# maiziezhoulab/FocalSV

Measured on AMD Instinct MI355X. Metric: target regions/sec (50 kb, 30x HiFi), higher is better.
Workload: dtype u32; 1 GPU; 256 synthetic 50 kb regions per GPU, 30x HiFi-like reads U(10k,20k), 0.2% error, seed 1000+i (BASELINE.json configs[1]); regions_per_gpu=256

## Files before the change

focalsv_amd/csrc/asm.hip:

```cpp
#include "asm_kernels.h"
#include "k_kmer.h"
#include "layout.h"
#include <algorithm>
#include <chrono>
#include <cstdio>
#include <cstdlib>
#include <cstring>
#include <vector>
#include <thread>
#include <atomic>

namespace {

enum { KN_SKETCH, KN_UNIQ, KN_CHAIN, KN_BPM, KN_RESCUE, KN_PATH_FAST, KN_PATH_DP, KN_CONSENSUS, KN_REPACK, KN_EXACT, KN_STITCH, KN_PARTITION, KN_BND, KN_BND_CONS,
       KN_UNIQ_LONG, KN_CHAIN_SPILL,
       KN_CONS_DEEP, KN_BND_DEEP,
       KN_COUNT,
       ST_SKETCH = KN_COUNT, ST_CHAIN, ST_VERIFY, ST_PATH, ST_CONSENSUS, ST_FINAL };
const char *const kn_names[KN_COUNT] = {"k_sketch", "k_uniq", "k_chain", "k5_bpm", "k_rescue_accept", "k_path_fast", "k_path_dp", "k_consensus",
                                        "k_repack", "k_exact", "k_stitch", "k_partition", "k_bnd_tasks", "k_bnd_consensus", "k_uniq_long", "k_chain_spill",
                                        "k_consensus_deep", "k_bnd_consensus_deep"};
static_assert(KN_COUNT <= FSV_MAX_KERNEL_STATS, "fsv_asm_stats holds every kernel's row");
enum { PASS_NONE = -1, PASS_WINDOWS, PASS_JUNCTIONS, PASS_BCIG, PASS_COUNT };

// ... 910 lines not shown
    BcigArgs BA;
    BA.tasks = W.tasks.p; BA.paths = W.paths.p; BA.n_tasks = R.ct + CT_TASKS;
    BA.pair_read = W.pair_read.p; BA.read_dirty = W.read_dirty.p; BA.gwin_off = W.gwin_off.p;
    BA.thr_tab = W.thr_tab.p; BA.k_cap = P.k_cap;
    BA.tasks2 = W.tasks2.p; BA.bc_idx = W.bc_idx.p; BA.n_tasks2 = ct3 + CT_TASKS;
    BA.n_same = ct3 + CT_B_RETRY; BA.n_used = ct3 + CT_B_LIST;
    BA.res2 = W.res2.p; BA.paths2 = W.paths2.p; BA.bc_rec = W.bc_rec.p; BA.bc_win = W.bc_win.p;
    W.kt.begin(ctx, KN_PARTITION, 0);
    FSV_LAUNCH(ctx, ctx->stream, k_bcig_tasks, dim3((fsv_grid_for(task_cap, 256) + 7u) & ~7u), dim3(256), 0, BA);
    W.kt.end(ctx);
    W.kt.begin(ctx, PASS_BCIG, KN_BPM, 0);
    TRY(fsv_bpm_windows_dev_n(ctx, R.store, W.tasks2.p, task_cap, ct3 + CT_TASKS, W.res2.p, P.k_cap));
    W.kt.end(ctx);
    TRY(path_stage(ctx, W, PathJob{R.store, W.tasks2.p, W.res2.p, W.paths2.p, task_cap, ct3 + CT_TASKS, ct3, PASS_BCIG, R.round, R.wide_bands, P.k_cap, false}));
    W.kt.begin(ctx, KN_PARTITION, 0);
    FSV_LAUNCH(ctx, ctx->stream, k_bcig_accept, dim3(fsv_grid_for(task_cap, 256)), dim3(256), 0, BA);
    W.kt.end(ctx);
    SA.bc_idx = W.bc_idx.p; SA.bc_rec = W.bc_rec.p; SA.bc_paths = W.paths2.p;
    SL.bc_win = W.bc_win.p;
    return FSV_OK;
}

static int consensus_stage(fsv_ctx *ctx, AsmWs &W, Round &R)
{
    const fsv_asm_params &P = R.P; const Batch &B = R.B;
    const uint32_t n_gwin = R.n_gwin;
    TRY(consensus_setup(ctx, W, R));
    const ConsArgs &C = R.C;
    const bool partition = B.n_pairs && P.partition;
    SiteArgs SA{};
    SiteLists SL{};
    if (partition) TRY(partition_setup(ctx, W, R, SA, SL));
    if (partition && P.junction_cigars) TRY(junction_cigars(ctx, W, R, SA, SL));
    const dim3 grid_w((n_gwin + 7u) & ~7u);
    W.kt.begin(ctx, PASS_WINDOWS, KN_CONSENSUS, (uint64_t)n_gwin * (96 + 448));
    if (R.wide_bands) {
        if (partition) FSV_LAUNCH(ctx, ctx->stream, (k_consensus<FSV_EV_CAP_WIDE, 1>), grid_w, dim3(64), 0, C, n_gwin, SL);
        else FSV_LAUNCH(ctx, ctx->stream, (k_consensus<FSV_EV_CAP_WIDE, 0>), grid_w, dim3(64), 0, C, n_gwin, SL);
    } else {
        if (partition) FSV_LAUNCH(ctx, ctx->stream, (k_consensus<FSV_EV_CAP, 1>), grid_w, dim3(64), 0, C, n_gwin, SL);
        else FSV_LAUNCH(ctx, ctx->stream, (k_consensus<FSV_EV_CAP, 0>), grid_w, dim3(64), 0, C, n_gwin, SL);
    }
    W.kt.end(ctx);
    if (partition) {
        const uint32_t grid_l = std::min<uint32_t>(std::max(1u, n_gwin), (uint32_t)ctx->n_cu * 16);
        W.kt.begin(ctx, KN_PARTITION, (uint64_t)B.n_reads * 4);
        FSV_LAUNCH(ctx, ctx->stream, k_snp_sites, dim3(grid_l), dim3(64), 0, C, SA, SL);
        FSV_LAUNCH(ctx, ctx->stream, k_hap_partition, dim3(B.n_reads), dim3(64), 0, C, SA, W.ovl.p, W.ovl_c.p, SL);
        if (R.wide_bands) FSV_LAUNCH(ctx, ctx->stream, k_consensus_redo<FSV_EV_CAP_WIDE>, dim3(grid_l), dim3(64), 0, C, SL);
        else FSV_LAUNCH(ctx, ctx->stream, k_consensus_redo<FSV_EV_CAP>, dim3(grid_l), dim3(64), 0, C, SL);
        W.kt.end(ctx);
    }
    if (C.deep_list) {
        W.kt.begin(ctx, KN_CONS_DEEP, 0);
        FSV_LAUNCH(ctx, ctx->stream, k_consensus_deep, dim3(R.deep_grid), dim3(64), 0, C, SL, R.deep);
        W.kt.end(ctx);
    }
    return FSV_OK;
}

static int finish_round(fsv_ctx *ctx, AsmWs &W, Round &R)
{
    const fsv_asm_params &P = R.P; const Batch &B = R.B;
    const uint32_t n_gwin = R.n_gwin;
    TRY(ensure(ctx, W.lb, std::max(1u, n_gwin)));
    FSV_LAUNCH(ctx, ctx->stream, k_newlen, dim3(fsv_grid_for(B.n_reads, 256)), dim3(256), 0, W.gwin_off.p, W.cwin_len.p, B.n_reads, W.new_len.p, W.lb.p);
    std::vector<int32_t> nlen(B.n_reads);
    TRY(download(ctx, nlen.data(), W.new_len, B.n_reads));
    for (int pass = 0; pass < PASS_COUNT; pass++)
        FSV_HIP(ctx, hipMemcpyAsync(R.h_ct.data() + (size_t)R.row(pass) * CT_SLOT, W.ct_of(R.row(pass)), CT_SLOT * 4, hipMemcpyDeviceToHost, ctx->stream));
    FSV_HIP(ctx, hipStreamSynchronize(ctx->stream));
    if (R.h_ct[(size_t)R.round * CT_SLOT + CT_OVERFLOW]) return fsv_fail(ctx, FSV_ECAP, "internal window task buffer overflow");
    Geometry G2;
    TRY(make_geometry(ctx, B, nlen, G2, P.w, &R.mz_fixed));
    Dev<uint32_t> &dst = W.store[R.round & 1];
    const uint32_t total_words = G2.word_off[B.n_reads];
    TRY(ensure(ctx, dst, (size_t)total_words + 8));
    TRY(upload(ctx, W.unpack_off, G2.word_off));
    W.kt.begin(ctx, KN_REPACK, (uint64_t)n_gwin * 384 + (uint64_t)total_words * 4);
    FSV_LAUNCH(ctx, ctx->stream, k_repack, dim3(B.n_reads), dim3(256), 0, W.gwin_off.p, W.lb.p, W.cwin.p, W.unpack_off.p, W.new_len.p, B.n_reads,
               R.round + 1 < P.n_rounds ? 1 : 0, dst.p);
    W.kt.end(ctx);
    FSV_HIP(ctx, hipMemsetAsync(dst.p + total_words, 0, 32, ctx->stream));
    R.store = dst.p;
    R.len = nlen;
    for (int32_t l : R.len) if (l >= 65536) R.short_reads = false;
    R.G = G2;
    return FSV_OK;
}

struct SetLayout { std::vector<std::vector<Piece>> contigs; bool fallback = false; };
struct Final {
    std::vector<uint32_t> hit_first, hwarn, h_setcols;
    const fsv_hit *hraw = nullptr;
    bool any_inexact = false;
    std::vector<SetLayout> lay;
    uint64_t used = 0;
    Trace trace;
};

static int begin_final(fsv_ctx *ctx, AsmWs &W, Round &R)
{
    R.ct = W.ct_of(R.P.n_rounds); R.task_cap = 0;
    TRY(upload(ctx, W.word_off, R.G.word_off));
    TRY(upload(ctx, W.len, R.len));
    TRY(upload(ctx, W.mz_off, R.G.mz_off));
    TRY(ensure(ctx, W.tasks, 2));
    return FSV_OK;
}

static int rechain_listed(fsv_ctx *ctx, AsmWs &W, const Round &R, const uint32_t *n_list_dev)
{
    const fsv_asm_params &P = R.P; const Batch &B = R.B;
    ChainArgs A2 = W.last_chain;
// ... 1036 lines not shown
```

focalsv_amd/csrc/asm_kernels.h:

```cpp
#pragma once
#include "bpm_device.h"
#include "k_sketch.h"
#include <type_traits>

#define FSV_AMAX       1024
#define FSV_AMAX_WIDE_LONG 2560
#define FSV_AMAX_WIDE  4096
#define FSV_PATH_CAP    416
#define FSV_CW_STRIDE   448
#define FSV_INS_MAXLEN   12
#define FSV_SB_MAXERR    7
#define FSV_SB_QUADS ((FSV_WINDOW + 3) / 4)
#define FSV_FR_MAXERR    3
#define FSV_EV_CAP_WIDE 2048
#define FSV_EV_CAP     256

static_assert(sizeof(fsv_wpath) == 128, "fsv_wpath layout");

namespace {


struct ChainArgs {
    const uint32_t *store;
    const uint32_t *word_off;
// ... 1514 lines not shown
        int lm0 = w.row >> 5, lm1 = lm0, lm2 = lm0, lm3 = lm0;
        ld(c0, lm0, lo0, hi0); ld(c0 - 1, lm1, lo1, hi1); ld(c0 - 2, lm2, lo2, hi2); ld(c0 - 3, lm3, lo3, hi3);
        for (int c = c0; c >= 0; c -= 4) {
            if (!__any(w.cur != 0 && w.ci >= 0 && fits)) break;
            column(c, lo0, hi0, lm0);
            column(c - 1, lo1, hi1, lm1);
            column(c - 2, lo2, hi2, lm2);
            column(c - 3, lo3, hi3, lm3);
        }
        w.flush();
        if (!fits) { T.P->state = 0; continue; }
        path_finish(store, T.t, T.P, w, T.end, T.err);
    }
}

}
#include "k_consensus.h"
namespace {

__global__ void k_newlen(const uint32_t *__restrict__ gwin_off, const uint16_t *__restrict__ cwin_len, uint32_t n_reads, int32_t *__restrict__ new_len,
                         uint32_t *__restrict__ lb = nullptr)
{
    const uint32_t r = blockIdx.x * blockDim.x + threadIdx.x;
    if (r >= n_reads) return;
    int32_t L = 0;
    for (uint32_t g = gwin_off[r]; g < gwin_off[r + 1]; g++) { if (lb) lb[g] = (uint32_t)L; L += cwin_len[g]; }
    new_len[r] = L;
}

#define FSV_RP_WIN 1024
__global__ __launch_bounds__(256) void k_repack(const uint32_t *__restrict__ gwin_off, const uint32_t *__restrict__ lb,
                                                const uint8_t *__restrict__ cwin, const uint32_t *__restrict__ new_word_off,
                                                const int32_t *__restrict__ new_len, uint32_t n_reads, int rc,
                                                uint32_t *__restrict__ out, const uint32_t *__restrict__ only = nullptr)
{
    __shared__ int s_lb[FSV_RP_WIN + 1];
    const uint32_t r = blockIdx.x;
    if (r >= n_reads) return;
    if (only && !only[r]) return;
    const uint32_t g0 = gwin_off[r], nw = gwin_off[r + 1] - g0;
    const int len = new_len[r];
    const uint32_t w0 = new_word_off[r], slot = new_word_off[r + 1] - w0;
    const bool in_lds = nw <= FSV_RP_WIN;
    if (in_lds) {
        for (uint32_t i = threadIdx.x; i < nw; i += 256) s_lb[i] = (int)lb[g0 + i];
        if (threadIdx.x == 0) s_lb[nw] = len;
    }
    __syncthreads();
    auto LB = [&](uint32_t i) -> int { return in_lds ? s_lb[i] : (i < nw ? (int)lb[g0 + i] : len); };
    for (uint32_t w = threadIdx.x; w < slot; w += 256) {
        const int b0 = (int)w * 16;
        uint32_t v = 0;
        if (b0 < len && nw) {
            int src = rc ? len - 1 - b0 : b0;
            uint32_t g = 0, hi = nw;
            while (hi - g > 1) { const uint32_t mid = (g + hi) >> 1; if (LB(mid) <= src) g = mid; else hi = mid; }
            for (int j = 0; j < 16 && b0 + j < len; j++) {
                uint32_t code = cwin[(size_t)(g0 + g) * FSV_CW_STRIDE + (src - LB(g))];
                if (rc) {
                    code = 3u - code;
                    src--;
                    while (g > 0 && src < LB(g)) g--;
                } else {
                    src++;
                    while (g + 1 < nw && src >= LB(g + 1)) g++;
                }
                v |= code << (2 * j);
            }
        }
        out[w0 + w] = v;
    }
}

struct fsv_hit { uint32_t q, t; int32_t x_s, x_e, y_s, y_e; uint32_t rev, slot; };

// ... 110 lines not shown
```

focalsv_amd/csrc/k_consensus.h:

```cpp
#pragma once

namespace {

struct ConsArgs {
    const uint32_t *store;
    const uint32_t *word_off;
    const int32_t *read_len;
    const uint32_t *read_set;
    const uint32_t *set_start;
    const uint32_t *pair_base;
    const uint32_t *gwin_off;
    const uint32_t *gwin_read;
    const uint4 *ovl_c;
    const uint4 *gwin_tab;
    const fsv_wtask *tasks;
    const fsv_wpath *paths;
    uint8_t *cwin;
    uint16_t *cwin_len;
    uint32_t *warn;
    uint32_t *changed;
    uint32_t n_reads;
    const uint32_t *read_dirty;
    uint8_t *cov3;
    int junction_vote;
// ... 301 lines not shown

template <class F>
__device__ __forceinline__ bool homo_strict(F B, int site, int len)
{
    const int beg = max(0, site - 3), end = min(len - 1, site + 3);
    const uint32_t own = B(site);
    uint32_t f_ch = 4u, b_ch = 4u;
    int f_len = 0, b_len = 0;
    for (int i = site + 1; i <= end; i++) {
        const uint32_t v = B(i);
        if (f_ch == 4u) { f_ch = v; f_len = 1; } else if (v != f_ch) break; else f_len++;
    }
    for (int i = site - 1; i >= beg; i--) {
        const uint32_t v = B(i);
        if (b_ch == 4u) { b_ch = v; b_len = 1; } else if (v != b_ch) break; else b_len++;
    }
    if (f_ch == own) f_len++;
    else if (b_ch == own) b_len++;
    return f_len >= 3 || b_len >= 3 || (own == f_ch && b_ch == f_ch && f_len + b_len >= 3);
}

__device__ __forceinline__ void load_path_ops(const fsv_wpath *P, uint2 (&pv)[13])
{
    const uint2 *src = reinterpret_cast<const uint2 *>(P->ops);
#pragma unroll
    for (int i = 0; i < 13; i++) pv[i] = src[i];
}
__device__ __forceinline__ void lane_columns(int lane, int n, int &c0, int &c1)
{
    const int per = (n + 63) / 64;
    c0 = min(n, lane * per); c1 = min(n, c0 + per);
}

struct TallyCols {
    uint32_t cnt[FSV_WINDOW + 1][3];
    int32_t cov[FSV_WINDOW + 2];
    uint32_t path[64][27];
    uint32_t xraw[28];
    uint32_t cover;

    __device__ __forceinline__ void reset(int lane)
    {
        for (int i = lane; i < (FSV_WINDOW + 1) * 3; i += 64) (&cnt[0][0])[i] = 0;
        for (int i = lane; i < FSV_WINDOW + 2; i += 64) cov[i] = 0;
        if (lane == 0) cover = 0;
    }
    __device__ __forceinline__ void stage_backbone(int lane, const uint32_t *__restrict__ x, int org, int len)
    {
        if (lane < 28) { const int wi = (org >> 4) - 1 + lane; xraw[lane] = (wi >= 0 && wi <= ((len + 15) >> 4)) ? x[wi] : 0u; }
    }
    __device__ __forceinline__ uint32_t xb(int org, int p) const { return (xraw[(p >> 4) - ((org >> 4) - 1)] >> ((p & 15) << 1)) & 3u; }
    __device__ __forceinline__ void cnt_add(int c, uint32_t b) { atomicAdd(&cnt[c][b >> 1], 1u << ((b & 1u) << 4)); }
    __device__ __forceinline__ uint32_t cnt_get(int c, uint32_t b) const { return (cnt[c][b >> 1] >> ((b & 1u) << 4)) & 0xffffu; }
    __device__ __forceinline__ uint32_t stage_path(int lane, const uint2 (&pv)[13])
    {
        uint32_t nz = 0;
#pragma unroll
        for (int i = 0; i < 13; i++) {
            path[lane][2 * i] = pv[i].x; path[lane][2 * i + 1] = pv[i].y;
            nz |= (pv[i].x ? 1u << (2 * i) : 0u) | (pv[i].y ? 2u << (2 * i) : 0u);
        }
        return nz;
    }
};

__device__ __forceinline__ bool split_sub_site(const int oa[4], int occ2, int arrived, int &alt)
{
    const int occ1 = oa[0] + oa[1] + oa[2] + oa[3];
    if (occ1 <= 1) return false;
    const int occ0 = arrived - occ1 - occ2;
    int mx = occ2;
    alt = -1;
#pragma unroll
    for (int b = 0; b < 4; b++) if (oa[b] > mx) { mx = oa[b]; alt = b; }
    if (occ0 == 0 || alt < 0 || mx <= 1) return false;
#pragma unroll
    for (int b = 0; b < 4; b++) if (oa[b] == mx && b != alt) return false;
    return (double)(occ0 + 1 + mx) / (double)(arrived + 1) >= 0.95 && (double)mx / (double)(arrived + 1 - (occ0 + 1)) >= 0.70;
}

template <class EV>
struct Tally : TallyCols {
    uint32_t evhead[FSV_WINDOW + 1];
// ... 176 lines not shown
                if (L <= FSV_INS_MAXLEN) {
                    const uint32_t e = (uint32_t)xp | ((uint32_t)(p - n3) << 9) | ((uint32_t)L << 19);
                    if (np == 0) ent[0] = e; else if (np == 1) ent[1] = e; else if (np == 2) ent[2] = e; else ent[3] = e;
                    np++;
                }
            }
            n2 += L; p += L;
            continue;
        }
        const bool after_ins = pend && p > 0;
        if (pend) { atomicAdd(&S.cnt[xp][2], 1u << 16); pend = false; }
        if (op == 3u) { atomicAdd(&S.cnt[xp][2], 1u); n3++; }
        else if (op == 1u) {
            const bool flagged = after_ins || fmm_pos == p;
            const uint32_t e = (uint32_t)xp | ((uint32_t)(p - n3) << 9) | (flagged ? 1u << 23 : 0u);
            if (np == 0) ent[0] = e; else if (np == 1) ent[1] = e; else if (np == 2) ent[2] = e; else ent[3] = e;
            np++;
            if (flagged) fmm_pos = p + 1;
        } else if (after_ins) fstart = xp;
        p++;
    }
    if (fstart >= 0) { atomicAdd(&S.cov[fstart], 65536); atomicAdd(&S.cov[xs + plen - n2], -65536); }
    if (np) cons_flush(S, store, y_word, y_len, y_rev, ry_start, ent, np);
    return n2;
}

struct SiteLists {
    uint32_t *site_cnt;
    uint32_t *win_list;
    uint32_t *redo_list;
    uint32_t *win_n;
    const int32_t *bc_win;
};
template <class EV, int MODE>
__device__ __forceinline__ void consensus_window(const ConsArgs &A, const uint32_t gw, const SiteLists &L, const EvSlab *slab = nullptr)
{
    __shared__ Tally<EV> S;
    __shared__ uint32_t s_anydev;
    const int lane = threadIdx.x;
    const uint4 gt = A.gwin_tab[gw];
    const uint32_t r = gt.x, pbase = gt.y, n_ovl = gt.z;
    const int g = (int)gt.w;
    const int xlen = A.read_len[r];
    const int gs = g * FSV_WINDOW, glen = min(FSV_WINDOW, xlen - gs);
    S.stage_backbone(lane, A.store + A.word_off[r], gs, xlen);
    uint8_t *dst = A.cwin + (size_t)gw * FSV_CW_STRIDE;
    if (A.read_dirty && !A.read_dirty[r]) {
        __syncthreads();
        for (int c = lane; c < glen; c += 64) dst[c] = (uint8_t)S.xb(gs, gs + c);
        if (lane == 0) { A.cwin_len[gw] = (uint16_t)glen; if (MODE == 1) L.site_cnt[gw] = 0u; }
        return;
    }
    S.reset(lane);
    if constexpr (EV::deep) { if (lane == 0) S.ev = *slab; }
    if (lane == 0) s_anydev = 0;
    __syncthreads();
    for (uint32_t oi = lane; oi < n_ovl; oi += 64) {
        const uint4 oc = A.ovl_c[pbase + oi];
        const int o_x_s = (int)oc.x, o_n_win = (int)(oc.z & 0x7fffffffu);
        const int j = g - o_x_s / FSV_WINDOW;
        if (!(oc.z >> 31) || j < 0 || j >= o_n_win) continue;
        const uint32_t ti = oc.y + (uint32_t)j;
        const fsv_wpath *P = A.paths + ti;
        const uint4 h0 = *reinterpret_cast<const uint4 *>(P);
        const uint2 h1 = *reinterpret_cast<const uint2 *>((const uint8_t *)P + 16);
        uint2 pv[13];
        load_path_ops(P, pv);
        atomicAdd(&S.cover, 1u);
        if ((h0.w & 0xffu) != 1u) continue;
        const bool clean_path = (int16_t)(h0.z >> 16) == 0;
        const uint32_t nz = clean_path ? 0u : S.stage_path(lane, pv);
        const int ry_start = (int)h0.x, plen = (int)(int16_t)(h0.z & 0xffffu);
        const uint32_t y_word = h1.x; const int y_len = (int)h1.y, y_rev = (int)((h0.w >> 8) & 0xffu);
        const int xs = max(gs, o_x_s) - gs;
        bool pend = false;
        if (j > 0 && A.junction_vote) {
            const uint4 hp = *reinterpret_cast<const uint4 *>(A.paths + ti - 1);
            if ((hp.w & 0xffu) == 1u) {
                const int gap = ry_start - (int)hp.y - 1;
                if (gap > 0 && xs == 0) {
                    pend = true;
                    if (gap <= FSV_INS_MAXLEN) {
                        uint32_t key = (uint32_t)gap << 24;
                        for (int b = 0; b < gap; b++) key |= fsv_base_at(A.store, y_word, y_len, y_rev, ry_start - gap + b) << (2 * b);
                        S.add_event(0, key);
                    }
                }
            }
        }
        if (pend || nz) s_anydev = 1u;
        int n2 = 0;
        if (clean_path) { if (pend) S.cnt_add(xs, 5u); }
        else n2 = cons_walk(S, S.path[lane], nz, plen, xs, glen, pend, A.store, y_word, y_len, y_rev, ry_start);
        atomicAdd(&S.cov[xs], 1);
        atomicAdd(&S.cov[xs + plen - n2], -1);
    }
    __syncthreads();
    const bool verbatim = S.cover < 3u || s_anydev == 0u;
    if (A.cov3 && lane == 0) A.cov3[gw] = S.cover >= 3u ? 1 : 0;
    if constexpr (!EV::deep) {
        if (lane == 0 && (S.evn > S.ev.cap() || (A.deep_list && S.cover > 255u))) {
            if (!A.deep_list) atomicOr(&A.warn[r], (uint32_t)FSV_W_INS_EVENTS);
            else if (!verbatim) deep_push(A.deep_list, A.deep_n, A.deep_cap, gw, S.evn);
        }
    }
    const int bc_lo = (MODE == 1 && L.bc_win) ? L.bc_win[3 * (size_t)gw + 1] : 1, bc_hi = (MODE == 1 && L.bc_win) ? L.bc_win[3 * (size_t)gw + 2] : 0;
    bool site = false;
    int c0, c1;
    lane_columns(lane, glen, c0, c1);
    const bool differs = S.decide_columns(lane, c0, c1, gs, glen, xlen, verbatim, A.ins_dag, [&](int c, int arrived, bool) {
        if (MODE != 1) return;
        int oa[4], alt;
#pragma unroll
        for (int b = 0; b < 4; b++) oa[b] = (int)S.cnt_get(c, (uint32_t)b);
        if (oa[0] + oa[1] + oa[2] + oa[3] > 1 && c >= bc_lo && c <= bc_hi) site = true;
        if (split_sub_site(oa, (int)S.cnt_get(c, 4u), arrived, alt)) site = true;
    });
    if (differs && A.changed) A.changed[r] = 1u;
    if (MODE == 1) {
        const bool any_site = __ballot(site) != 0ull || (L.bc_win && L.bc_win[3 * (size_t)gw]);
        if (lane == 0) {
            L.site_cnt[gw] = any_site ? FSV_SITE_MARK : 0u;
            if (any_site) L.win_list[atomicAdd(&L.win_n[0], 1u)] = gw;
        }
    }
    uint8_t (*s_out)[14] = S.out();
    uint32_t mine = 0;
    for (int c = c0; c < c1; c++) mine += s_out[c][0];
    const int incl = wave_incl_sum((int)mine, lane);
    uint32_t off = (uint32_t)incl - mine;
    const uint32_t tot = (uint32_t)__shfl(incl, 63, 64);
    if (tot > FSV_CW_STRIDE) {
        for (int c = lane; c < glen; c += 64) dst[c] = (uint8_t)S.xb(gs, gs + c);
        if (lane == 0) { A.cwin_len[gw] = (uint16_t)glen; atomicOr(&A.warn[r], (uint32_t)FSV_W_WINDOW_KEPT); }
        return;
    }
    for (int c = c0; c < c1; c++) for (int b = 0; b < s_out[c][0]; b++) dst[off++] = s_out[c][1 + b];
    if (lane == 0) A.cwin_len[gw] = (uint16_t)tot;
}

template <int EVC, int MODE>
__global__ __launch_bounds__(64) void k_consensus(ConsArgs A, uint32_t n_gwin, SiteLists L)
{
    uint32_t gw;
    if (xcd_block(n_gwin, gw)) consensus_window<EvLds<EVC>, MODE>(A, gw, L);
}

template <int EVC>
__global__ __launch_bounds__(64) void k_consensus_redo(ConsArgs A, SiteLists L)
{
    const uint32_t n = L.win_n[1];
    for (uint32_t i = blockIdx.x; i < n; i += gridDim.x) {
        consensus_window<EvLds<EVC>, 0>(A, L.redo_list[i], L);
        __syncthreads();
    }
}

struct DeepSlabs {
    uint32_t *base; uint32_t cap;
    uint32_t *max_events;
    __device__ __forceinline__ EvSlab of_block(uint32_t b) const
    {
        uint32_t *p = base + (size_t)b * 3u * cap;
        return EvSlab{p, p + cap, p + 2 * (size_t)cap, cap};
    }
};
__global__ __launch_bounds__(64) void k_consensus_deep(ConsArgs A, SiteLists L, DeepSlabs D)
{
    const uint32_t n = min(*A.deep_n, A.deep_cap);
    const EvSlab ev = D.of_block(blockIdx.x);
    for (uint32_t i = blockIdx.x; i < n; i += gridDim.x) {
        const uint2 e = A.deep_list[i];
        if (threadIdx.x == 0) atomicMax(D.max_events, e.y);
        consensus_window<EvSlab, 0>(A, e.x, L, &ev);
        __syncthreads();
    }
}

#define FSV_BC_SIDE 100
#define FSV_BC_USELESS 50
#define FSV_BC_SCAN 10
struct BcigArgs {
    const fsv_wtask *tasks; const fsv_wpath *paths; const uint32_t *n_tasks;
    const uint32_t *pair_read, *read_dirty, *gwin_off; const uint8_t *thr_tab; int k_cap;
    fsv_wtask *tasks2; int32_t *bc_idx; uint32_t *n_tasks2;
    const fsv_wres *res2; const fsv_wpath *paths2; uint4 *bc_rec; int32_t *bc_win;
    uint32_t *n_same, *n_used;
};
struct OpReader {
    const uint32_t *w; uint32_t cur = 0; int idx = -1;
    __device__ __forceinline__ OpReader(const fsv_wpath *P) : w(reinterpret_cast<const uint32_t *>(P->ops)) {}
    __device__ __forceinline__ uint32_t get(int i) { const int wi = i >> 4; if (wi != idx) { cur = w[wi]; idx = wi; } return (cur >> ((i & 15) << 1)) & 3u; }
};
__device__ __forceinline__ int scan_ops(const fsv_wpath *P, int plen, int err0, int scan_x, int dir)
{
    if (err0 == 0) return 0;
    OpReader R(P);
    int x_i = 0, err = 0;
    for (int p = 0; p < plen; p++) {
        const uint32_t op = R.get(dir ? plen - 1 - p : p);
        if (op == 2u) { err++; continue; }
        if (op != 0u) err++;
        if (++x_i >= scan_x) return err;
    }
    return err;
}
__device__ __forceinline__ int scan_ops_interval(const fsv_wpath *P, int plen, int err0, int xb, int xe)
// ... 532 lines not shown
    w.x_len = (uint16_t)blen; w.k = A.thr_tab[blen]; w.y_rev = t.y_rev; w.ovl = p; w.win = ti;
    A.tasks2[slot] = w;
    A.idx2[ti] = (int32_t)slot;
    if (!(atomicOr(&A.bnd_flag[gw], 1u) & 1u)) A.bnd_list[atomicAdd(A.n_bnd, 1u)] = gw;
}

__global__ __launch_bounds__(256) void k_bnd_retry(fsv_wtask *__restrict__ tasks2, const fsv_wres *__restrict__ res2, const uint32_t *__restrict__ n_tasks2,
                                                   fsv_wtask *__restrict__ tasks3, uint32_t *__restrict__ src3, uint32_t *__restrict__ n3, int k_cap)
{
    const uint32_t i = blockIdx.x * blockDim.x + threadIdx.x;
    if (i >= *n_tasks2 || res2[i].err >= 0) return;
    fsv_wtask t = tasks2[i];
    t.k = (uint8_t)double_thr(t.k, t.x_len, k_cap);
    tasks2[i].k = t.k;
    const uint32_t j = atomicAdd(n3, 1u);
    tasks3[j] = t; src3[j] = i;
}

__global__ __launch_bounds__(256) void k_bnd_scatter(fsv_wres *__restrict__ res2, const fsv_wres *__restrict__ res3, const uint32_t *__restrict__ src3,
                                                     const uint32_t *__restrict__ n3)
{
    const uint32_t j = blockIdx.x * blockDim.x + threadIdx.x;
    if (j < *n3) res2[src3[j]] = res3[j];
}

struct BndPatch { uint16_t ts, told, tnew, hs, hold, hnew, valid, pad; };

template <class EV>
struct BndLds : Tally<EV> {
    uint32_t terr;
    uint16_t off[FSV_WINDOW + 2];
    uint8_t own[FSV_WINDOW + 1];
};
template <class EV, bool SPILL>
__device__ __forceinline__ void bnd_junction(const ConsArgs &A, const BndArgs &B, const fsv_wpath *__restrict__ paths2, const uint32_t *__restrict__ store2,
                                             BndPatch *__restrict__ patch, uint8_t *__restrict__ patch_bytes, const uint32_t gw, const EvSlab *slab = nullptr)
{
    static_assert(2 * FSV_BND_HALF + 1 <= FSV_WINDOW, "a junction's backbone fits the tally of a window");
    __shared__ BndLds<EV> S;
    const int lane = threadIdx.x;
    const uint4 gt = A.gwin_tab[gw];
    const uint32_t r = gt.x, pbase = gt.y, n_ovl = gt.z;
    const int g = (int)gt.w;
    const int gs = g * FSV_WINDOW;
    const int LB = (int)B.lb[gw], len_now = LB + (int)B.cwin_len[gw];
    const int cws = max(0, LB - FSV_BND_HALF), cwe = min(len_now - 1, LB + FSV_BND_HALF - 1), blen = cwe - cws + 1;
    if (lane == 0) { patch[gw].valid = 0; S.terr = 0; }
    S.stage_backbone(lane, store2 + B.b_base + B.brel_off[r], cws, len_now);
    S.reset(lane);
    if constexpr (EV::deep) { if (lane == 0) S.ev = *slab; }
    __syncthreads();
    for (uint32_t oi = lane; oi < n_ovl; oi += 64) {
        const uint4 oc = A.ovl_c[pbase + oi];
        const int o_x_s = (int)oc.x, o_n_win = (int)(oc.z & 0x7fffffffu);
        const int j = g - o_x_s / FSV_WINDOW;
        if (!(oc.z >> 31) || j < 0 || j >= o_n_win || o_x_s > gs) continue;
        const int32_t slot = B.idx2[oc.y + (uint32_t)j];
        if (slot == -2) { atomicAdd(&S.cover, 1u); atomicAdd(&S.cov[0], 1); atomicAdd(&S.cov[blen], -1); continue; }
        if (slot < 0) continue;
        const fsv_wpath *P = paths2 + slot;
        const uint4 h0 = *reinterpret_cast<const uint4 *>(P);
        if ((h0.w & 0xffu) != 1u) continue;
        const uint2 h1 = *reinterpret_cast<const uint2 *>((const uint8_t *)P + 16);
        const int perr = (int)(int16_t)(h0.z >> 16);
        atomicAdd(&S.cover, 1u);
        const int ry_start = (int)h0.x, plen = (int)(int16_t)(h0.z & 0xffffu);
        int n2 = 0;
        if (perr != 0) {
            atomicAdd(&S.terr, (uint32_t)perr);
            uint2 pv[13];
            load_path_ops(P, pv);
            const uint32_t nz = S.stage_path(lane, pv);
            n2 = cons_walk(S, S.path[lane], nz, plen, 0, blen, false, A.store, h1.x, (int)h1.y, (int)((h0.w >> 8) & 0xffu), ry_start);
        }
        atomicAdd(&S.cov[0], 1);
        atomicAdd(&S.cov[plen - n2], -1);
    }
    __syncthreads();
    if (S.cover < 3u || S.terr == 0u) return;
    if constexpr (!EV::deep) {
        if (lane == 0 && (S.evn > S.ev.cap() || (SPILL && S.cover > 255u))) {
            if (!SPILL) atomicOr(&A.warn[r], (uint32_t)FSV_W_INS_EVENTS);
            else deep_push(B.deep_list, B.deep_n, B.deep_cap, gw, S.evn);
        }
    }
    int c0, c1;
    lane_columns(lane, blen, c0, c1);
    for (int c = c0; c < c1; c++) S.own[c] = 1;
    const bool differs = S.decide_columns(lane, c0, c1, cws, blen, len_now, false, A.ins_dag, [&](int c, int, bool kept) { S.own[c] = kept; });
    uint8_t (*s_out)[14] = S.out();
    int mine = 0;
    for (int c = c0; c < c1; c++) mine += s_out[c][0];
    if (__ballot(differs) == 0ull) return;
    int off = wave_incl_sum(mine, lane) - mine;
    for (int c = c0; c < c1; c++) { S.off[c] = (uint16_t)off; off += s_out[c][0]; }
    const int sb = FSV_BND_SIDE, eb = blen - 1 - FSV_BND_SIDE;
    int fs = 0x7fffffff, fe = 0x7fffffff;
    for (int c = c0; c < c1; c++) { if (S.own[c] && c >= sb && c < fs) fs = c; if (S.own[c] && c >= eb && c < fe) fe = c; }
    for (int d = 32; d >= 1; d >>= 1) { fs = min(fs, __shfl_xor(fs, d)); fe = min(fe, __shfl_xor(fe, d)); }
    __syncthreads();
    if (eb <= sb || fs == 0x7fffffff || fe == 0x7fffffff) return;
    const int o0 = (int)S.off[fs] + s_out[fs][0] - 1, o1 = (int)S.off[fe] + s_out[fe][0] - 1;
    const int R0 = cws + fs, R1 = cws + fe, sc = LB - cws;
    const int o_split = sc <= fs ? o0 : (sc > fe ? o1 + 1 : (int)S.off[sc]);
    const int lb_prev = (int)B.lb[gw - 1];
    BndPatch bp;
    bp.valid = 1; bp.pad = 0;
    bp.ts = (uint16_t)max(0, R0 - lb_prev); bp.told = (uint16_t)max(0, min(R1, LB - 1) - R0 + 1); bp.tnew = (uint16_t)(o_split - o0);
    bp.hs = (uint16_t)(max(R0, LB) - LB); bp.hold = (uint16_t)max(0, R1 - max(R0, LB) + 1); bp.hnew = (uint16_t)(o1 + 1 - o_split);
    if (R0 < lb_prev || o1 + 1 - o0 > FSV_CW_STRIDE) {
        if (lane == 0) atomicOr(&A.warn[r], (uint32_t)FSV_W_WINDOW_KEPT);
        return;
    }
    uint8_t *dst = patch_bytes + (size_t)gw * FSV_CW_STRIDE;
    for (int c = c0; c < c1; c++)
        for (int b = 0; b < s_out[c][0]; b++) { const int pos = (int)S.off[c] + b; if (pos >= o0 && pos <= o1) dst[pos - o0] = s_out[c][1 + b]; }
    if (lane == 0) patch[gw] = bp;
}

template <int EVC, bool SPILL>
__global__ __launch_bounds__(64) void k_bnd_consensus(ConsArgs A, BndArgs B, const fsv_wpath *__restrict__ paths2, const uint32_t *__restrict__ store2,
                                                      BndPatch *__restrict__ patch, uint8_t *__restrict__ patch_bytes)
{
    const uint32_t n_list = *B.n_bnd;
    for (uint32_t li = blockIdx.x; li < n_list; li += gridDim.x) {
        __syncthreads();
        bnd_junction<EvLds<EVC>, SPILL>(A, B, paths2, store2, patch, patch_bytes, B.bnd_list[li]);
    }
}

__global__ __launch_bounds__(64) void k_bnd_consensus_deep(ConsArgs A, BndArgs B, const fsv_wpath *__restrict__ paths2, const uint32_t *__restrict__ store2,
                                                           BndPatch *__restrict__ patch, uint8_t *__restrict__ patch_bytes, DeepSlabs D)
{
    const uint32_t n = min(*B.deep_n, B.deep_cap);
    const EvSlab ev = D.of_block(blockIdx.x);
    for (uint32_t i = blockIdx.x; i < n; i += gridDim.x) {
        __syncthreads();
        const uint2 e = B.deep_list[i];
        if (threadIdx.x == 0) atomicMax(D.max_events, e.y);
        bnd_junction<EvSlab, false>(A, B, paths2, store2, patch, patch_bytes, e.x, &ev);
    }
}

__global__ __launch_bounds__(64) void k_bnd_apply(const uint32_t *__restrict__ gwin_read, const uint32_t *__restrict__ gwin_off, const BndPatch *__restrict__ patch,
                                                  const uint8_t *__restrict__ patch_bytes, const uint32_t *__restrict__ bnd_flag, uint32_t n_gwin,
                                                  uint8_t *__restrict__ cwin, uint16_t *__restrict__ cwin_len, uint32_t *__restrict__ changed, uint32_t *__restrict__ warn)
{
    __shared__ uint8_t s_old[FSV_CW_STRIDE];
    const uint32_t gw = blockIdx.x;
    if (gw >= n_gwin) return;
    const uint32_t r = gwin_read[gw];
    const bool has_h = gw > gwin_off[r] && (bnd_flag[gw] & 1u) && patch[gw].valid;
    const bool has_t = gw + 1 < gwin_off[r + 1] && (bnd_flag[gw + 1] & 1u) && patch[gw + 1].valid;
    if (!has_h && !has_t) return;
    const int lane = threadIdx.x;
    const int len = cwin_len[gw];
    uint8_t *w = cwin + (size_t)gw * FSV_CW_STRIDE;
    for (int i = lane; i < len; i += 64) s_old[i] = w[i];
    __syncthreads();
    int hs = 0, hold = 0, hnew = 0, ts = len, told = 0, tnew = 0;
    const uint8_t *hb = nullptr, *tb = nullptr;
    if (has_h) { const BndPatch p = patch[gw]; hs = p.hs; hold = p.hold; hnew = p.hnew; hb = patch_bytes + (size_t)gw * FSV_CW_STRIDE + p.tnew; }
    if (has_t) { const BndPatch p = patch[gw + 1]; ts = p.ts; told = p.told; tnew = p.tnew; tb = patch_bytes + (size_t)(gw + 1) * FSV_CW_STRIDE; }
    if (told == 0 && tnew == 0) ts = len;
    const int new_len = len - hold + hnew - told + tnew;
    if (hs + hold > ts || ts + told > len || new_len > FSV_CW_STRIDE || new_len < 0) {
        if (lane == 0) atomicOr(&warn[r], (uint32_t)FSV_W_WINDOW_KEPT);
        return;
    }
    const int a1 = hs, a2 = a1 + hnew, a3 = a2 + (ts - hs - hold), a4 = a3 + tnew;
    for (int i = lane; i < new_len; i += 64) {
        uint8_t v;
        if (i < a1) v = s_old[i];
// ... 11 lines not shown
```

Measured before the change: 2521 regions/s.

## Chunk consensus windows per block with prefetch and skip clean-read window copies

```diff
diff --git a/focalsv_amd/csrc/asm.hip b/focalsv_amd/csrc/asm.hip
--- a/focalsv_amd/csrc/asm.hip
+++ b/focalsv_amd/csrc/asm.hip
@@ -966,7 +966,7 @@
     SiteLists SL{};
     if (partition) TRY(partition_setup(ctx, W, R, SA, SL));
     if (partition && P.junction_cigars) TRY(junction_cigars(ctx, W, R, SA, SL));
-    const dim3 grid_w((n_gwin + 7u) & ~7u);
+    const dim3 grid_w(((n_gwin + FSV_CONS_CH - 1) / FSV_CONS_CH + 7u) & ~7u);
     W.kt.begin(ctx, PASS_WINDOWS, KN_CONSENSUS, (uint64_t)n_gwin * (96 + 448));
     if (R.wide_bands) {
         if (partition) FSV_LAUNCH(ctx, ctx->stream, (k_consensus<FSV_EV_CAP_WIDE, 1>), grid_w, dim3(64), 0, C, n_gwin, SL);
@@ -1013,7 +1013,7 @@
     TRY(upload(ctx, W.unpack_off, G2.word_off));
     W.kt.begin(ctx, KN_REPACK, (uint64_t)n_gwin * 384 + (uint64_t)total_words * 4);
     FSV_LAUNCH(ctx, ctx->stream, k_repack, dim3(B.n_reads), dim3(256), 0, W.gwin_off.p, W.lb.p, W.cwin.p, W.unpack_off.p, W.new_len.p, B.n_reads,
-               R.round + 1 < P.n_rounds ? 1 : 0, dst.p);
+               R.round + 1 < P.n_rounds ? 1 : 0, dst.p, (const uint32_t *)nullptr, R.store, W.word_off.p, R.C.read_dirty);
     W.kt.end(ctx);
     FSV_HIP(ctx, hipMemsetAsync(dst.p + total_words, 0, 32, ctx->stream));
     R.store = dst.p;
diff --git a/focalsv_amd/csrc/asm_kernels.h b/focalsv_amd/csrc/asm_kernels.h
--- a/focalsv_amd/csrc/asm_kernels.h
+++ b/focalsv_amd/csrc/asm_kernels.h
@@ -1570,7 +1570,9 @@
 __global__ __launch_bounds__(256) void k_repack(const uint32_t *__restrict__ gwin_off, const uint32_t *__restrict__ lb,
                                                 const uint8_t *__restrict__ cwin, const uint32_t *__restrict__ new_word_off,
                                                 const int32_t *__restrict__ new_len, uint32_t n_reads, int rc,
-                                                uint32_t *__restrict__ out, const uint32_t *__restrict__ only = nullptr)
+                                                uint32_t *__restrict__ out, const uint32_t *__restrict__ only = nullptr,
+                                                const uint32_t *__restrict__ old = nullptr, const uint32_t *__restrict__ old_word_off = nullptr,
+                                                const uint32_t *__restrict__ dirty = nullptr)
 {
     __shared__ int s_lb[FSV_RP_WIN + 1];
     const uint32_t r = blockIdx.x;
@@ -1579,6 +1581,20 @@
     const uint32_t g0 = gwin_off[r], nw = gwin_off[r + 1] - g0;
     const int len = new_len[r];
     const uint32_t w0 = new_word_off[r], slot = new_word_off[r + 1] - w0;
+    if (dirty && !dirty[r]) {
+        const uint32_t *src = old + old_word_off[r];
+        const int nwords = (len + 15) >> 4;
+        for (uint32_t w = threadIdx.x; w < slot; w += 256) {
+            const int b0 = (int)w * 16;
+            uint32_t v = 0;
+            if (b0 < len) {
+                v = rc ? ~rev_fields2(load_fwd16(src, nwords, len - 16 - b0)) : src[w];
+                if (len - b0 < 16) v &= (1u << (2 * (len - b0))) - 1u;
+            }
+            out[w0 + w] = v;
+        }
+        return;
+    }
     const bool in_lds = nw <= FSV_RP_WIN;
     if (in_lds) {
         for (uint32_t i = threadIdx.x; i < nw; i += 256) s_lb[i] = (int)lb[g0 + i];
diff --git a/focalsv_amd/csrc/k_consensus.h b/focalsv_amd/csrc/k_consensus.h
--- a/focalsv_amd/csrc/k_consensus.h
+++ b/focalsv_amd/csrc/k_consensus.h
@@ -357,6 +357,12 @@
     c0 = min(n, lane * per); c1 = min(n, c0 + per);
 }
 
+__device__ __forceinline__ uint32_t backbone_word(int lane, const uint32_t *__restrict__ x, int org, int len)
+{
+    const int wi = (org >> 4) - 1 + lane;
+    return (lane < 28 && wi >= 0 && wi <= ((len + 15) >> 4)) ? x[wi] : 0u;
+}
+
 struct TallyCols {
     uint32_t cnt[FSV_WINDOW + 1][3];
     int32_t cov[FSV_WINDOW + 2];
@@ -370,10 +376,8 @@
         for (int i = lane; i < FSV_WINDOW + 2; i += 64) cov[i] = 0;
         if (lane == 0) cover = 0;
     }
-    __device__ __forceinline__ void stage_backbone(int lane, const uint32_t *__restrict__ x, int org, int len)
-    {
-        if (lane < 28) { const int wi = (org >> 4) - 1 + lane; xraw[lane] = (wi >= 0 && wi <= ((len + 15) >> 4)) ? x[wi] : 0u; }
-    }
+    __device__ __forceinline__ void stage_backbone(int lane, const uint32_t *__restrict__ x, int org, int len) { put_backbone(lane, backbone_word(lane, x, org, len)); }
+    __device__ __forceinline__ void put_backbone(int lane, uint32_t word) { if (lane < 28) xraw[lane] = word; }
     __device__ __forceinline__ uint32_t xb(int org, int p) const { return (xraw[(p >> 4) - ((org >> 4) - 1)] >> ((p & 15) << 1)) & 3u; }
     __device__ __forceinline__ void cnt_add(int c, uint32_t b) { atomicAdd(&cnt[c][b >> 1], 1u << ((b & 1u) << 4)); }
     __device__ __forceinline__ uint32_t cnt_get(int c, uint32_t b) const { return (cnt[c][b >> 1] >> ((b & 1u) << 4)) & 0xffffu; }
@@ -616,59 +620,75 @@
     uint32_t *win_n;
     const int32_t *bc_win;
 };
+struct PathRec { uint4 h0; uint2 h1; uint2 pv[13]; };
+struct ReadView { uint32_t r, pbase, n_ovl, word_off; int xlen; bool clean; uint4 oc; };
+struct WinView { uint32_t xword; int j; uint4 hp; PathRec rec; };
+__device__ __forceinline__ void load_path_rec(const fsv_wpath *P, PathRec &R)
+{
+    R.h0 = *reinterpret_cast<const uint4 *>(P);
+    R.h1 = *reinterpret_cast<const uint2 *>((const uint8_t *)P + 16);
+    load_path_ops(P, R.pv);
+}
+__device__ __forceinline__ int ovl_window(const uint4 &oc, int g)
+{
+    const int j = g - (int)oc.x / FSV_WINDOW;
+    return ((oc.z >> 31) && j >= 0 && j < (int)(oc.z & 0x7fffffffu)) ? j : -1;
+}
+__device__ __forceinline__ void load_read_ovl(const ConsArgs &A, int lane, ReadView &V)
+{
+    V.oc = (uint32_t)lane < V.n_ovl ? A.ovl_c[V.pbase + (uint32_t)lane] : make_uint4(0, 0, 0, 0);
+}
+__device__ __forceinline__ void load_window(const ConsArgs &A, const ReadView &V, int g, int lane, bool with_prev, WinView &W)
+{
+    W.xword = backbone_word(lane, A.store + V.word_off, g * FSV_WINDOW, V.xlen);
+    W.j = ovl_window(V.oc, g);
+    W.hp = make_uint4(0, 0, 0, 0);
+    if (W.j >= 0) {
+        const fsv_wpath *P = A.paths + (V.oc.y + (uint32_t)W.j);
+        load_path_rec(P, W.rec);
+        if (with_prev && W.j > 0 && A.junction_vote) W.hp = *reinterpret_cast<const uint4 *>(P - 1);
+    }
+}
+
 template <class EV, int MODE>
-__device__ __forceinline__ void consensus_window(const ConsArgs &A, const uint32_t gw, const SiteLists &L, const EvSlab *slab = nullptr)
+__device__ __forceinline__ void consensus_window(const ConsArgs &A, const uint32_t gw, const int g, const ReadView &V, const WinView &W,
+                                                 const SiteLists &L, const EvSlab *slab = nullptr)
 {
     __shared__ Tally<EV> S;
     __shared__ uint32_t s_anydev;
     const int lane = threadIdx.x;
-    const uint4 gt = A.gwin_tab[gw];
-    const uint32_t r = gt.x, pbase = gt.y, n_ovl = gt.z;
-    const int g = (int)gt.w;
-    const int xlen = A.read_len[r];
+    const uint32_t r = V.r;
+    const int xlen = V.xlen;
     const int gs = g * FSV_WINDOW, glen = min(FSV_WINDOW, xlen - gs);
-    S.stage_backbone(lane, A.store + A.word_off[r], gs, xlen);
     uint8_t *dst = A.cwin + (size_t)gw * FSV_CW_STRIDE;
-    if (A.read_dirty && !A.read_dirty[r]) {
-        __syncthreads();
-        for (int c = lane; c < glen; c += 64) dst[c] = (uint8_t)S.xb(gs, gs + c);
+    if (V.clean) {
         if (lane == 0) { A.cwin_len[gw] = (uint16_t)glen; if (MODE == 1) L.site_cnt[gw] = 0u; }
         return;
     }
+    S.put_backbone(lane, W.xword);
     S.reset(lane);
     if constexpr (EV::deep) { if (lane == 0) S.ev = *slab; }
     if (lane == 0) s_anydev = 0;
     __syncthreads();
-    for (uint32_t oi = lane; oi < n_ovl; oi += 64) {
-        const uint4 oc = A.ovl_c[pbase + oi];
-        const int o_x_s = (int)oc.x, o_n_win = (int)(oc.z & 0x7fffffffu);
-        const int j = g - o_x_s / FSV_WINDOW;
-        if (!(oc.z >> 31) || j < 0 || j >= o_n_win) continue;
-        const uint32_t ti = oc.y + (uint32_t)j;
-        const fsv_wpath *P = A.paths + ti;
-        const uint4 h0 = *reinterpret_cast<const uint4 *>(P);
-        const uint2 h1 = *reinterpret_cast<const uint2 *>((const uint8_t *)P + 16);
-        uint2 pv[13];
-        load_path_ops(P, pv);
+    auto vote = [&](const uint4 &oc, int j, const PathRec &R, const uint4 &hp) {
+        const int o_x_s = (int)oc.x;
+        const uint4 h0 = R.h0;
         atomicAdd(&S.cover, 1u);
-        if ((h0.w & 0xffu) != 1u) continue;
+        if ((h0.w & 0xffu) != 1u) return;
         const bool clean_path = (int16_t)(h0.z >> 16) == 0;
-        const uint32_t nz = clean_path ? 0u : S.stage_path(lane, pv);
+        const uint32_t nz = clean_path ? 0u : S.stage_path(lane, R.pv);
         const int ry_start = (int)h0.x, plen = (int)(int16_t)(h0.z & 0xffffu);
-        const uint32_t y_word = h1.x; const int y_len = (int)h1.y, y_rev = (int)((h0.w >> 8) & 0xffu);
+        const uint32_t y_word = R.h1.x; const int y_len = (int)R.h1.y, y_rev = (int)((h0.w >> 8) & 0xffu);
         const int xs = max(gs, o_x_s) - gs;
         bool pend = false;
-        if (j > 0 && A.junction_vote) {
-            const uint4 hp = *reinterpret_cast<const uint4 *>(A.paths + ti - 1);
-            if ((hp.w & 0xffu) == 1u) {
-                const int gap = ry_start - (int)hp.y - 1;
-                if (gap > 0 && xs == 0) {
-                    pend = true;
-                    if (gap <= FSV_INS_MAXLEN) {
-                        uint32_t key = (uint32_t)gap << 24;
-                        for (int b = 0; b < gap; b++) key |= fsv_base_at(A.store, y_word, y_len, y_rev, ry_start - gap + b) << (2 * b);
-                        S.add_event(0, key);
-                    }
+        if (j > 0 && A.junction_vote && (hp.w & 0xffu) == 1u) {
+            const int gap = ry_start - (int)hp.y - 1;
+            if (gap > 0 && xs == 0) {
+                pend = true;
+                if (gap <= FSV_INS_MAXLEN) {
+                    uint32_t key = (uint32_t)gap << 24;
+                    for (int b = 0; b < gap; b++) key |= fsv_base_at(A.store, y_word, y_len, y_rev, ry_start - gap + b) << (2 * b);
+                    S.add_event(0, key);
                 }
             }
         }
@@ -678,6 +698,17 @@
         else n2 = cons_walk(S, S.path[lane], nz, plen, xs, glen, pend, A.store, y_word, y_len, y_rev, ry_start);
         atomicAdd(&S.cov[xs], 1);
         atomicAdd(&S.cov[xs + plen - n2], -1);
+    };
+    if (W.j >= 0) vote(V.oc, W.j, W.rec, W.hp);
+    for (uint32_t oi = lane + 64; oi < V.n_ovl; oi += 64) {
+        const uint4 oc = A.ovl_c[V.pbase + oi];
+        const int j = ovl_window(oc, g);
+        if (j < 0) continue;
+        const fsv_wpath *P = A.paths + (oc.y + (uint32_t)j);
+        PathRec R;
+        load_path_rec(P, R);
+        const uint4 hp = (j > 0 && A.junction_vote) ? *reinterpret_cast<const uint4 *>(P - 1) : make_uint4(0, 0, 0, 0);
+        vote(oc, j, R, hp);
     }
     __syncthreads();
     const bool verbatim = S.cover < 3u || s_anydev == 0u;
@@ -723,11 +754,68 @@
     if (lane == 0) A.cwin_len[gw] = (uint16_t)tot;
 }
 
+template <class EV, int MODE>
+__device__ __forceinline__ void consensus_window_at(const ConsArgs &A, const uint32_t gw, const SiteLists &L, const EvSlab *slab = nullptr)
+{
+    const int lane = threadIdx.x;
+    const uint4 gt = A.gwin_tab[gw];
+    ReadView V;
+    V.r = gt.x; V.pbase = gt.y; V.n_ovl = gt.z;
+    V.xlen = A.read_len[V.r]; V.word_off = A.word_off[V.r];
+    V.clean = A.read_dirty && !A.read_dirty[V.r];
+    load_read_ovl(A, lane, V);
+    WinView W;
+    W.j = -1;
+    if (!V.clean) load_window(A, V, (int)gt.w, lane, true, W);
+    consensus_window<EV, MODE>(A, gw, (int)gt.w, V, W, L, slab);
+}
+
+#define FSV_CONS_CH 8
 template <int EVC, int MODE>
 __global__ __launch_bounds__(64) void k_consensus(ConsArgs A, uint32_t n_gwin, SiteLists L)
 {
-    uint32_t gw;
-    if (xcd_block(n_gwin, gw)) consensus_window<EvLds<EVC>, MODE>(A, gw, L);
+    const int lane = threadIdx.x;
+    uint32_t chunk;
+    if (!xcd_block((n_gwin + FSV_CONS_CH - 1) / FSV_CONS_CH, chunk)) return;
+    const uint32_t first = chunk * FSV_CONS_CH;
+    const int nw = (int)min((uint32_t)FSV_CONS_CH, n_gwin - first);
+    uint4 gtv = make_uint4(0xffffffffu, 0, 0, 0);
+    int xlen_v = 0;
+    uint32_t woff_v = 0, clean_v = 0;
+    if (lane < nw) {
+        gtv = A.gwin_tab[first + lane];
+        xlen_v = A.read_len[gtv.x]; woff_v = A.word_off[gtv.x];
+        clean_v = (A.read_dirty && !A.read_dirty[gtv.x]) ? 1u : 0u;
+    }
+    ReadView V;
+    V.r = 0xffffffffu; V.clean = true;
+    WinView cur, nxt;
+    cur.j = -1; nxt.j = -1;
+    bool have_cur = false;
+#pragma nounroll
+    for (int k = 0; k < nw; k++) {
+#define RL(v_, k_) ((uint32_t)__builtin_amdgcn_readlane((int)(v_), k_))
+        const uint32_t gw = first + (uint32_t)k, r = RL(gtv.x, k);
+        const int g = (int)RL(gtv.w, k);
+        if (r != V.r) {
+            V.r = r; V.pbase = RL(gtv.y, k); V.n_ovl = RL(gtv.z, k);
+            V.xlen = (int)RL(xlen_v, k); V.word_off = RL(woff_v, k); V.clean = RL(clean_v, k) != 0u;
+            if (!V.clean) load_read_ovl(A, lane, V);
+            have_cur = false;
+        }
+        const bool have_nxt = !V.clean && k + 1 < nw && RL(gtv.x, min(k + 1, FSV_CONS_CH - 1)) == r;
+#undef RL
+        if (!V.clean) {
+            if (!have_cur) load_window(A, V, g, lane, true, cur);
+            if (have_nxt) {
+                load_window(A, V, g + 1, lane, false, nxt);
+                if (cur.j >= 0) nxt.hp = cur.rec.h0;
+            }
+        }
+        consensus_window<EvLds<EVC>, MODE>(A, gw, g, V, cur, L);
+        __syncthreads();
+        cur = nxt; have_cur = have_nxt;
+    }
 }
 
 template <int EVC>
@@ -735,7 +823,7 @@
 {
     const uint32_t n = L.win_n[1];
     for (uint32_t i = blockIdx.x; i < n; i += gridDim.x) {
-        consensus_window<EvLds<EVC>, 0>(A, L.redo_list[i], L);
+        consensus_window_at<EvLds<EVC>, 0>(A, L.redo_list[i], L);
         __syncthreads();
     }
 }
@@ -756,7 +844,7 @@
     for (uint32_t i = blockIdx.x; i < n; i += gridDim.x) {
         const uint2 e = A.deep_list[i];
         if (threadIdx.x == 0) atomicMax(D.max_events, e.y);
-        consensus_window<EvSlab, 0>(A, e.x, L, &ev);
+        consensus_window_at<EvSlab, 0>(A, e.x, L, &ev);
         __syncthreads();
     }
 }
@@ -1355,50 +1443,87 @@
     uint16_t off[FSV_WINDOW + 2];
     uint8_t own[FSV_WINDOW + 1];
 };
-template <class EV, bool SPILL>
+struct JuncView {
+    uint32_t gw; int stage;
+    uint4 gt; uint32_t lb, cwl;
+    uint32_t brel; uint4 oc;
+    uint32_t xword; int32_t slot;
+    PathRec rec;
+    __device__ __forceinline__ int LB() const { return (int)lb; }
+    __device__ __forceinline__ int len_now() const { return (int)lb + (int)cwl; }
+    __device__ __forceinline__ int cws() const { return max(0, (int)lb - FSV_BND_HALF); }
+};
+__device__ __forceinline__ int32_t junc_slot(const BndArgs &B, const uint4 &oc, int g)
+{
+    const int j = ovl_window(oc, g);
+    return (j >= 0 && (int)oc.x <= g * FSV_WINDOW) ? B.idx2[oc.y + (uint32_t)j] : -1;
+}
+__device__ __forceinline__ void junc_advance(const ConsArgs &A, const BndArgs &B, const fsv_wpath *__restrict__ paths2, const uint32_t *__restrict__ store2,
+                                             int lane, JuncView &J, int upto)
+{
+    if (J.stage < 1 && upto >= 1) {
+        J.gt = A.gwin_tab[J.gw]; J.lb = B.lb[J.gw]; J.cwl = B.cwin_len[J.gw];
+        J.stage = 1;
+    }
+    if (J.stage < 2 && upto >= 2) {
+        J.brel = B.brel_off[J.gt.x];
+        J.oc = (uint32_t)lane < J.gt.z ? A.ovl_c[J.gt.y + (uint32_t)lane] : make_uint4(0, 0, 0, 0);
+        J.stage = 2;
+    }
+    if (J.stage < 3 && upto >= 3) {
+        J.xword = backbone_word(lane, store2 + B.b_base + J.brel, J.cws(), J.len_now());
+        J.slot = junc_slot(B, J.oc, (int)J.gt.w);
+        J.stage = 3;
+    }
+    if (J.stage < 4 && upto >= 4) {
+        if (J.slot >= 0) load_path_rec(paths2 + J.slot, J.rec);
+        J.stage = 4;
+    }
+}
+
+template <class EV, bool SPILL, class F>
 __device__ __forceinline__ void bnd_junction(const ConsArgs &A, const BndArgs &B, const fsv_wpath *__restrict__ paths2, const uint32_t *__restrict__ store2,
-                                             BndPatch *__restrict__ patch, uint8_t *__restrict__ patch_bytes, const uint32_t gw, const EvSlab *slab = nullptr)
+                                             BndPatch *__restrict__ patch, uint8_t *__restrict__ patch_bytes, const JuncView &J, F between,
+                                             const EvSlab *slab = nullptr)
 {
     static_assert(2 * FSV_BND_HALF + 1 <= FSV_WINDOW, "a junction's backbone fits the tally of a window");
     __shared__ BndLds<EV> S;
     const int lane = threadIdx.x;
-    const uint4 gt = A.gwin_tab[gw];
-    const uint32_t r = gt.x, pbase = gt.y, n_ovl = gt.z;
-    const int g = (int)gt.w;
-    const int gs = g * FSV_WINDOW;
-    const int LB = (int)B.lb[gw], len_now = LB + (int)B.cwin_len[gw];
-    const int cws = max(0, LB - FSV_BND_HALF), cwe = min(len_now - 1, LB + FSV_BND_HALF - 1), blen = cwe - cws + 1;
+    const uint32_t gw = J.gw, r = J.gt.x, pbase = J.gt.y, n_ovl = J.gt.z;
+    const int g = (int)J.gt.w;
+    const int LB = J.LB(), len_now = J.len_now();
+    const int cws = J.cws(), cwe = min(len_now - 1, LB + FSV_BND_HALF - 1), blen = cwe - cws + 1;
     if (lane == 0) { patch[gw].valid = 0; S.terr = 0; }
-    S.stage_backbone(lane, store2 + B.b_base + B.brel_off[r], cws, len_now);
+    S.put_backbone(lane, J.xword);
     S.reset(lane);
     if constexpr (EV::deep) { if (lane == 0) S.ev = *slab; }
+    between(1);
     __syncthreads();
-    for (uint32_t oi = lane; oi < n_ovl; oi += 64) {
-        const uint4 oc = A.ovl_c[pbase + oi];
-        const int o_x_s = (int)oc.x, o_n_win = (int)(oc.z & 0x7fffffffu);
-        const int j = g - o_x_s / FSV_WINDOW;
-        if (!(oc.z >> 31) || j < 0 || j >= o_n_win || o_x_s > gs) continue;
-        const int32_t slot = B.idx2[oc.y + (uint32_t)j];
-        if (slot == -2) { atomicAdd(&S.cover, 1u); atomicAdd(&S.cov[0], 1); atomicAdd(&S.cov[blen], -1); continue; }
-        if (slot < 0) continue;
-        const fsv_wpath *P = paths2 + slot;
-        const uint4 h0 = *reinterpret_cast<const uint4 *>(P);
-        if ((h0.w & 0xffu) != 1u) continue;
-        const uint2 h1 = *reinterpret_cast<const uint2 *>((const uint8_t *)P + 16);
+    auto vote = [&](int32_t slot, const PathRec &R) {
+        if (slot == -2) { atomicAdd(&S.cover, 1u); atomicAdd(&S.cov[0], 1); atomicAdd(&S.cov[blen], -1); return; }
+        if (slot < 0) return;
+        const uint4 h0 = R.h0;
+        if ((h0.w & 0xffu) != 1u) return;
         const int perr = (int)(int16_t)(h0.z >> 16);
         atomicAdd(&S.cover, 1u);
         const int ry_start = (int)h0.x, plen = (int)(int16_t)(h0.z & 0xffffu);
         int n2 = 0;
         if (perr != 0) {
             atomicAdd(&S.terr, (uint32_t)perr);
-            uint2 pv[13];
-            load_path_ops(P, pv);
-            const uint32_t nz = S.stage_path(lane, pv);
-            n2 = cons_walk(S, S.path[lane], nz, plen, 0, blen, false, A.store, h1.x, (int)h1.y, (int)((h0.w >> 8) & 0xffu), ry_start);
+            const uint32_t nz = S.stage_path(lane, R.pv);
+            n2 = cons_walk(S, S.path[lane], nz, plen, 0, blen, false, A.store, R.h1.x, (int)R.h1.y, (int)((h0.w >> 8) & 0xffu), ry_start);
         }
         atomicAdd(&S.cov[0], 1);
         atomicAdd(&S.cov[plen - n2], -1);
-    }
+    };
+    vote(J.slot, J.rec);
+    for (uint32_t oi = lane + 64; oi < n_ovl; oi += 64) {
+        const int32_t slot = junc_slot(B, A.ovl_c[pbase + oi], g);
+        PathRec R;
+        if (slot >= 0) load_path_rec(paths2 + slot, R);
+        vote(slot, R);
+    }
+    between(2);
     __syncthreads();
     if (S.cover < 3u || S.terr == 0u) return;
     if constexpr (!EV::deep) {
@@ -1411,6 +1536,7 @@
     lane_columns(lane, blen, c0, c1);
     for (int c = c0; c < c1; c++) S.own[c] = 1;
     const bool differs = S.decide_columns(lane, c0, c1, cws, blen, len_now, false, A.ins_dag, [&](int c, int, bool kept) { S.own[c] = kept; });
+    between(3);
     uint8_t (*s_out)[14] = S.out();
     int mine = 0;
     for (int c = c0; c < c1; c++) mine += s_out[c][0];
@@ -1445,10 +1571,22 @@
 __global__ __launch_bounds__(64) void k_bnd_consensus(ConsArgs A, BndArgs B, const fsv_wpath *__restrict__ paths2, const uint32_t *__restrict__ store2,
                                                       BndPatch *__restrict__ patch, uint8_t *__restrict__ patch_bytes)
 {
-    const uint32_t n_list = *B.n_bnd;
-    for (uint32_t li = blockIdx.x; li < n_list; li += gridDim.x) {
-        __syncthreads();
-        bnd_junction<EvLds<EVC>, SPILL>(A, B, paths2, store2, patch, patch_bytes, B.bnd_list[li]);
+    const int lane = threadIdx.x;
+    const uint32_t n_list = *B.n_bnd, G = gridDim.x;
+    uint32_t li = blockIdx.x;
+    if (li >= n_list) return;
+    JuncView cur, nxt;
+    cur.gw = B.bnd_list[li]; cur.stage = 0;
+    uint32_t gw_n = li + G < n_list ? B.bnd_list[li + G] : 0u;
+    for (; li < n_list; li += G) {
+        junc_advance(A, B, paths2, store2, lane, cur, 4);
+        const bool have_n = li + G < n_list;
+        nxt.gw = gw_n; nxt.stage = 0;
+        if (li + 2 * (uint64_t)G < n_list) gw_n = B.bnd_list[li + 2 * G];
+        __syncthreads();
+        bnd_junction<EvLds<EVC>, SPILL>(A, B, paths2, store2, patch, patch_bytes, cur,
+                                        [&](int k) { if (have_n) junc_advance(A, B, paths2, store2, lane, nxt, k); });
+        cur = nxt;
     }
 }
 
@@ -1461,7 +1599,10 @@
         __syncthreads();
         const uint2 e = B.deep_list[i];
         if (threadIdx.x == 0) atomicMax(D.max_events, e.y);
-        bnd_junction<EvSlab, false>(A, B, paths2, store2, patch, patch_bytes, e.x, &ev);
+        JuncView J;
+        J.gw = e.x; J.stage = 0;
+        junc_advance(A, B, paths2, store2, (int)threadIdx.x, J, 4);
+        bnd_junction<EvSlab, false>(A, B, paths2, store2, patch, patch_bytes, J, [](int) {}, &ev);
     }
 }
 
```

Result: slower. 2372 regions/s (-5.9%).
